# Hunger-Prevails/3D-Pose-Estimation-with-Previleged-Information

Measured on AMD Instinct MI355X. Metric: crops/sec (fwd+bwd) ResNet-50 pose head, 256x256 bs=64/GPU, higher is better.
Workload: dtype f32 (3xbf16 split, 6 products, f32 accumulate); 1 GPU; depthnet resnet50 pose head, 256x256 crops, batch 64/GPU, full step: fwd + soft-argmax + SmoothL1 + bwd + RCCL grad all-reduce + clip + Adam; global_batch=64, parallelism=dp1, dist_world_size=1, wgrad_stream_runs_beside_launch_stream=True

## Files before the change

### 3d-pose-estimation-with-previleged-information_amd/csrc/p3d_fx.hip

```cpp
#include <type_traits>
#include <mutex>
#include "p3d_common.h"
#include "p3d_fx.h"

namespace p3d {

using bf8 = __bf16 __attribute__((ext_vector_type(8)));
using f32x16 = float __attribute__((ext_vector_type(16)));
using f32x4 = float __attribute__((ext_vector_type(4)));
using f32x2 = float __attribute__((ext_vector_type(2)));
using u32x2 = unsigned __attribute__((ext_vector_type(2)));
using s4t = short __attribute__((ext_vector_type(4)));
using s8v = short __attribute__((ext_vector_type(8)));
using i32x4 = int __attribute__((ext_vector_type(4)));

constexpr int FX_BM = 128, FX_BN = 128, FX_BK = 16;
constexpr int FX_PIECE = 128 * FX_BK * 2;

using bf16x2 = __bf16 __attribute__((ext_vector_type(2)));
__device__ __forceinline__ unsigned fx_pack2(float a, float b) {
    const bf16x2 h = __builtin_convertvector(f32x2{a, b}, bf16x2);
    return __builtin_bit_cast(unsigned, h);
}
__device__ __forceinline__ void fx_split2(float x0, float x1, unsigned& hp, unsigned& mp, unsigned& lp) {
    hp = fx_pack2(x0, x1);
    const float r0 = x0 - __builtin_bit_cast(float, hp << 16), r1 = x1 - __builtin_bit_cast(float, hp & 0xFFFF0000u);
    mp = fx_pack2(r0, r1);
    const float s0 = r0 - __builtin_bit_cast(float, mp << 16), s1 = r1 - __builtin_bit_cast(float, mp & 0xFFFF0000u);
    lp = fx_pack2(s0, s1);
}
__device__ __forceinline__ void fx_split_store(unsigned char* base, const f32x4 v) {
    unsigned hp[2], mp[2], lp[2];
#pragma unroll
    for (int q = 0; q < 2; ++q) fx_split2(v[2 * q], v[2 * q + 1], hp[q], mp[q], lp[q]);
    *reinterpret_cast<u32x2*>(base) = u32x2{hp[0], hp[1]};
    *reinterpret_cast<u32x2*>(base + FX_PIECE) = u32x2{mp[0], mp[1]};
    *reinterpret_cast<u32x2*>(base + 2 * FX_PIECE) = u32x2{lp[0], lp[1]};
}

__device__ __forceinline__ int fx_tr_off(int row, int ch) { return 256 * row + 16 * (ch ^ (((row & 3) << 2) | ((row >> 2) & 3))); }
__device__ __forceinline__ int fx_rc_off(int row, int half) { return 32 * row + 16 * (half ^ ((row >> 3) & 1)); }

#define P3D_FX_PRODUCTS_AB(ACC, PIX, CH, NA, NB) P3D_FX_PRODUCTS_RANGE(ACC, PIX, CH, NA, NB, 0, 6)
#define P3D_FX_PRODUCTS_RANGE(ACC, PIX, CH, NA, NB, P0, P1)                                                            \
    _Pragma("unroll") for (int pa = P0; pa < P1; ++pa) {                                                               \
        constexpr int PP[6] = {2, 0, 1, 1, 0, 0}, PC[6] = {0, 2, 1, 0, 1, 0};                                           \
        _Pragma("unroll") for (int a = 0; a < NA; ++a) _Pragma("unroll") for (int b = 0; b < NB; ++b)                   \
            ACC[a][b] = __builtin_amdgcn_mfma_f32_32x32x16_bf16(PIX[PP[pa]][a], CH[PC[pa]][b], ACC[a][b], 0, 0, 0);    \
    }
__device__ __forceinline__ int fx_live_subtiles(int first, int limit) {
    const int n = (limit - first + 31) >> 5;
    return __builtin_amdgcn_readfirstlane(n < 0 ? 0 : (n > 2 ? 2 : n));
}

constexpr int FX_OOB = (int)0x80000000;
#if (defined(P3D_FX_ABL_NOLOAD) || defined(P3D_FX_ABL_NOREAD) || defined(P3D_FX_ABL_NOSTAGE) || defined(P3D_FX_ABL_NOBAR)) && !defined(P3D_TIMING_ONLY_BUILD)
#error "P3D_FX_ABL_* builds compute wrong results: define P3D_TIMING_ONLY_BUILD as well (tools/ablate.sh does) and never ship the library"
#endif
#ifdef P3D_FX_ABL_NOLOAD
#define FX_SO(x) 0
#else
#define FX_SO(x) (x)
#endif
#ifdef P3D_FX_ABL_NOREAD
#define FX_ABL_READ(kt) ((kt) == 0)
#else
#define FX_ABL_READ(kt) true
#endif
__device__ f32x4 fx_buffer_load_f32x4(i32x4 rsrc, int voffset, int soffset, int aux) __asm("llvm.amdgcn.raw.buffer.load.v4f32");
__device__ i32x4 fx_buffer_load_i32x4(i32x4 rsrc, int voffset, int soffset, int aux) __asm("llvm.amdgcn.raw.buffer.load.v4i32");
__device__ float fx_buffer_load_f32(i32x4 rsrc, int voffset, int soffset, int aux) __asm("llvm.amdgcn.raw.buffer.load.f32");
__device__ __forceinline__ i32x4 fx_rsrc(const void* base, size_t bytes) {
    const unsigned n = bytes < (size_t)0x80000000u ? (unsigned)bytes : 0x80000000u;
    const uint64_t a = reinterpret_cast<uint64_t>(base);
    i32x4 r;
    r[0] = (int)(unsigned)a; r[1] = (int)((a >> 32) & 0xffff); r[2] = (int)n; r[3] = 0x00020000;
    return r;
}
__device__ __forceinline__ bf8 fx_tr_read(const unsigned char* base, const int (&off)[2]) {
    s8v v;
#pragma unroll
    for (int half = 0; half < 2; ++half) {
        const s4t r4 = __builtin_amdgcn_ds_read_tr16_b64_v4i16((__attribute__((address_space(3))) s4t*)(base + off[half]));
#pragma unroll
        for (int e = 0; e < 4; ++e) v[4 * half + e] = r4[e];
    }
    return __builtin_bit_cast(bf8, v);
}
__device__ __forceinline__ void fx_tr_frag_off(int lane, int cb, int (&off)[2]) {
    const int g = lane >> 4, idx = lane & 15, q = idx >> 2, pq = idx & 3;
#pragma unroll
    for (int half = 0; half < 2; ++half) {
        const int row = 8 * (g >> 1) + 4 * half + q;
        off[half] = fx_tr_off(row, ((cb + 16 * (g & 1)) >> 3) + (pq >> 1)) + 8 * (pq & 1);
    }
}

__device__ __forceinline__ FxConvParams fx_class_params(const FxConvParams& in) {
    FxConvParams p = in;
    if (in.ncls > 0) {
        const FxConvClass& c = in.cls[blockIdx.z];
        p.nR = c.nR; p.nS = c.nS; p.ntap = c.ntap; p.r0 = c.r0; p.rstep = c.rstep; p.s0 = c.s0; p.sstep = c.sstep;
        p.hoff = c.hoff; p.hstep = c.hstep; p.woff = c.woff; p.wstep = c.wstep; p.oy0 = c.oy0; p.ox0 = c.ox0;
    }
    return p;
}

template <int AMODE, int PRO, int EPIX, bool TAPI = false>
__global__ __launch_bounds__(256, 3) void fx_conv_kernel(const FxConvParams p_in) {
    static_assert(!TAPI || AMODE == 1, "the tap-inner K order is an image-fed instance");
    constexpr int EPI = EPIX == 5 ? 1 : EPIX == 6 ? 2 : EPIX == 7 || EPIX == 8 ? 0 : EPIX;
    constexpr bool EM = EPIX == 4 || (EPIX >= 5 && EPIX <= 7);
    const FxConvParams p = fx_class_params(p_in);
    static_assert(AMODE == 0 || PRO == 0, "the partial-convolution factor is applied by the in-kernel split");
    __shared__ __attribute__((aligned(16))) unsigned char lds[2 * 6 * FX_PIECE];
    constexpr int BUFB = 6 * FX_PIECE, CH0 = 3 * FX_PIECE;
    float (*const red)[2][128] = reinterpret_cast<float (*)[2][128]>(lds + 40960);
    const int t = threadIdx.x, lane = t & 63, wave = __builtin_amdgcn_readfirstlane(t >> 6), wm = wave >> 1, wn = wave & 1;
    int bid;
    {
        const int nwg = gridDim.x, q = nwg >> 3, r = nwg & 7, xcd = blockIdx.x & 7, idx = blockIdx.x >> 3;
        bid = (xcd < r ? xcd * (q + 1) : r * (q + 1) + (xcd - r) * q) + idx;
    }
    const int tiles_n_all = gridDim.x / p.tiles_m;
    const int tile_m = p.order ? bid / tiles_n_all : bid % p.tiles_m, tile_n = p.order ? bid % tiles_n_all : bid / p.tiles_m;
    const int m0 = tile_m * FX_BM, n0 = tile_n * FX_BN;
    const int OHW = p.OH * p.OW;
    const int HWi = p.Hi * p.Wi;
    const int nfirst = n0 / OHW;
    const int csteps = p.Cred / FX_BK;
    int nk = p.ntap * csteps, kt0 = 0;
    if (p.kchunk > 0) {
        kt0 = blockIdx.y * p.kchunk;
        nk = min(nk - kt0, p.kchunk);
    }
    int f_tap = kt0 / csteps, f_k = (kt0 - f_tap * csteps) * FX_BK;
    if constexpr (TAPI) { f_k = (kt0 / p.ntap) * FX_BK; f_tap = kt0 - (kt0 / p.ntap) * p.ntap; }

    const i32x4 rW = fx_rsrc(p.Wimg, (size_t)p.R * p.S * p.tiles_m * csteps * (3 * FX_PIECE));
    int w_voff[3];
#pragma unroll
    for (int j = 0; j < 3; ++j) w_voff[j] = 16 * (t + 256 * j);

    const int trow = t >> 5, tp4 = t & 31;
    const int pp = t >> 1, ph = (t & 1) ^ ((t >> 4) & 1);
    const int col = n0 + (AMODE == 0 ? 4 * tp4 : pp);
    const bool col_ok = col < p.NP;
    int hbase = 0, wbase = 0, img_off = 0, mimg_off = 0;
    {
        const int cc = col_ok ? col : 0;
        const int pn = cc / OHW;
        const int rem = cc - pn * OHW, oh = rem / p.OW, ow = rem - oh * p.OW;
        hbase = oh * p.hmul + p.hoff;
        wbase = ow * p.wmul + p.woff;
// ... 569 lines not shown
                    for (int e = 0; e < 4; ++e) dst[e * p.oxs] = p.accumulate ? dst[e * p.oxs] + v[e] : v[e];
                }
            }
            if constexpr (EPI == 1) {
                if (!split) {
#pragma unroll
                    for (int e = 0; e < 4; ++e) { ssum[b] += v[e]; ssq[b] = fmaf(v[e], v[e], ssq[b]); }
                }
            }
            if constexpr (EPI == 2) {
                if (!split) {
                    const f32x4 c2 = *reinterpret_cast<const f32x4*>(p.ep_c + ((size_t)n * p.M + m) * OHW + rem);
#pragma unroll
                    for (int e = 0; e < 4; ++e) {
                        const float gg = fmaf(c2[e], esc[b], esh[b]) > 0.f ? v[e] : 0.f;
                        ssum[b] += gg; ssq[b] = fmaf(gg, c2[e] - emean[b], ssq[b]);
                    }
                }
            }
        }
    }
    if (dense) {
        constexpr int EROW = 512 + 16;
        constexpr int ROUNDS = (GB + 1) / 2;
        const bool accum = !split && p.accumulate;
#pragma unroll
        for (int r = 0; r < ROUNDS; ++r) {
            if (r > 0) __syncthreads();
#pragma unroll
            for (int b2 = 0; b2 < 2; ++b2) {
                const int b = 2 * r + b2;
                if (b < GB) {
#pragma unroll
                    for (int a = 0; a < GA; ++a)
                        *reinterpret_cast<f32x4*>(lds + (wm * 32 + b2 * 16 + lc) * EROW + (wn * 64 + a * 16 + 4 * lq) * 4) = acc[a][b < GB ? b : 0];
                }
            }
            __syncthreads();
#pragma unroll
            for (int i = 0; i < 8; ++i) {
                const int id = t + 256 * i, row = id >> 5, q = id & 31;
                const int within = r * 32 + (row & 31);
                const int m = m0 + (row >> 5) * WCH + within;
                const int c4 = n0 + 4 * q;
                if (within >= WCH || m >= p.M || c4 >= p.NP) continue;
                const int n = c4 / OHW, rem = c4 - n * OHW;
                f32x4 v = *reinterpret_cast<const f32x4*>(lds + row * EROW + q * 16);
                const size_t at = ((size_t)n * p.M + m) * OHW + rem;
                f32x4* dst = reinterpret_cast<f32x4*>(yout + at);
                if (accum) {
                    f32x4 o4;
                    if (p.acc_src) {
                        o4 = *reinterpret_cast<const f32x4*>(p.acc_src + at);
                        if (p.acc_mask) {
                            const unsigned mk = p.acc_mask[at >> 2];
#pragma unroll
                            for (int e = 0; e < 4; ++e) o4[e] = (mk >> e) & 1u ? o4[e] : 0.f;
                        }
                    } else o4 = *dst;
                    v[0] += o4[0]; v[1] += o4[1]; v[2] += o4[2]; v[3] += o4[3];
                }
                if constexpr (EPI == 8) {
                    if (p.ep_res) { const f32x4 r4 = *reinterpret_cast<const f32x4*>(p.ep_res + at); v[0] += r4[0]; v[1] += r4[1]; v[2] += r4[2]; v[3] += r4[3]; }
                    if (p.ep_relu) { v[0] = fmaxf(v[0], 0.f); v[1] = fmaxf(v[1], 0.f); v[2] = fmaxf(v[2], 0.f); v[3] = fmaxf(v[3], 0.f); }
                }
                *dst = v;
            }
        }
    }
    if constexpr (EPI == 1 || EPI == 2) {
        if (!split) {
#pragma unroll
            for (int b = 0; b < GB; ++b) {
                ssum[b] += __shfl_xor(ssum[b], 16, 64); ssq[b] += __shfl_xor(ssq[b], 16, 64);
                ssum[b] += __shfl_xor(ssum[b], 32, 64); ssq[b] += __shfl_xor(ssq[b], 32, 64);
                if (lq == 0) { red[wn][0][wm * WCH + b * 16 + lc] = ssum[b]; red[wn][1][wm * WCH + b * 16 + lc] = ssq[b]; }
            }
            __syncthreads();
            if (t < BM && m0 + t < p.M) {
                float* dst = p.partial + ((size_t)tile_n * p.M + m0 + t) * 2;
                dst[0] = red[0][0][t] + red[1][0][t];
                dst[1] = red[0][1][t] + red[1][1][t];
            }
        }
    }
}

template <int EPI>
__global__ __launch_bounds__(256) void fx_reduce_kernel(const float* __restrict__ slabs, float* __restrict__ y, const float* __restrict__ bias, int nsplit,
                                                        size_t slab_stride, int N, int M, int OHW, int accumulate, const float* __restrict__ ep_c,
                                                        const float* __restrict__ ep_tab, float* __restrict__ partial, const float* __restrict__ emask,
                                                        const float* __restrict__ res, int relu) {
    const int m = blockIdx.x, grp = blockIdx.y, ngrp = gridDim.y;
    const float bb = bias ? bias[m] : 0.f;
    float esc = 0.f, esh = 0.f, emean = 0.f;
    if constexpr (EPI == 2) { esc = ep_tab[8 * m]; esh = ep_tab[8 * m + 1]; emean = ep_tab[8 * m + 2]; }
    float s1 = 0.f, s2 = 0.f;
    const int q4 = OHW >> 2;
    for (int n = grp; n < N; n += ngrp) {
        const size_t base = ((size_t)n * M + m) * OHW;
        for (int i = threadIdx.x; i < q4; i += 256) {
            f32x4 v = *reinterpret_cast<const f32x4*>(slabs + base + 4 * i);
            for (int z = 1; z < nsplit; ++z) {
                const f32x4 u = *reinterpret_cast<const f32x4*>(slabs + (size_t)z * slab_stride + base + 4 * i);
                v[0] += u[0]; v[1] += u[1]; v[2] += u[2]; v[3] += u[3];
            }
            v[0] += bb; v[1] += bb; v[2] += bb; v[3] += bb;
            if (emask) {
                const f32x4 em = *reinterpret_cast<const f32x4*>(emask + (size_t)n * OHW + 4 * i);
                v[0] *= em[0]; v[1] *= em[1]; v[2] *= em[2]; v[3] *= em[3];
            }
            f32x4* dst = reinterpret_cast<f32x4*>(y + base + 4 * i);
            if (accumulate) { const f32x4 o = *dst; v[0] += o[0]; v[1] += o[1]; v[2] += o[2]; v[3] += o[3]; }
            if (res) { const f32x4 r4 = *reinterpret_cast<const f32x4*>(res + base + 4 * i); v[0] += r4[0]; v[1] += r4[1]; v[2] += r4[2]; v[3] += r4[3]; }
            if (relu) { v[0] = fmaxf(v[0], 0.f); v[1] = fmaxf(v[1], 0.f); v[2] = fmaxf(v[2], 0.f); v[3] = fmaxf(v[3], 0.f); }
            *dst = v;
            if constexpr (EPI == 1) {
#pragma unroll
                for (int e = 0; e < 4; ++e) { s1 += v[e]; s2 = fmaf(v[e], v[e], s2); }
            }
            if constexpr (EPI == 2) {
                const f32x4 c2 = *reinterpret_cast<const f32x4*>(ep_c + base + 4 * i);
#pragma unroll
                for (int e = 0; e < 4; ++e) { const float gg = fmaf(c2[e], esc, esh) > 0.f ? v[e] : 0.f; s1 += gg; s2 = fmaf(gg, c2[e] - emean, s2); }
            }
        }
    }
    if constexpr (EPI != 0) {
        __shared__ float r1[4], r2[4];
        s1 = wave_sum(s1); s2 = wave_sum(s2);
        if ((threadIdx.x & 63) == 0) { r1[threadIdx.x >> 6] = s1; r2[threadIdx.x >> 6] = s2; }
        __syncthreads();
        if (threadIdx.x == 0) {
            float* dst = partial + ((size_t)grp * M + m) * 2;
            dst[0] = r1[0] + r1[1] + r1[2] + r1[3];
            dst[1] = r2[0] + r2[1] + r2[2] + r2[3];
        }
    }
}

template <bool AIMG, bool BIMG, bool MASKED, int TAPS = 0>
__global__ __launch_bounds__(256, 3) void fx_wgrad_kernel(const FxWgradParams p) {
    static_assert(TAPS < 2 || (AIMG && BIMG && !MASKED), "the multi-tap column tiles are image-fed instances");
    static_assert(!MASKED || !AIMG || !BIMG, "the partial-convolution factors are applied by the in-kernel split of an fp32 operand (an image carries its factor already)");
    static_assert(!TAPS || BIMG, "tap-major columns come from an image operand");
    __shared__ __attribute__((aligned(16))) unsigned char As[2 * 3 * FX_PIECE];
    __shared__ __attribute__((aligned(16))) unsigned char Bs[2 * 3 * FX_PIECE];
    const int t = threadIdx.x, lane = t & 63, wave = t >> 6, wm = wave >> 1, wn = wave & 1;
    int bx, by, bz;
    {
        const int gx = gridDim.x, gy = gridDim.y, nwg = gx * gy * gridDim.z;
        const int lin = blockIdx.x + gx * (blockIdx.y + gy * blockIdx.z);
        const int q = nwg >> 3, r = nwg & 7, xcd = lin & 7, idx = lin >> 3;
        const int bid = (xcd < r ? xcd * (q + 1) : r * (q + 1) + (xcd - r) * q) + idx;
        if (p.order == 0 || TAPS) {
            bx = bid % gx;
            const int rest = bid / gx;
            by = rest % gy;
            bz = rest / gy;
        } else {
            const int nt = p.R * p.S;
            const int tp = bid % nt;
            int rest = bid / nt;
            by = rest % gy; rest /= gy;
            bx = rest % gx;
            bz = (rest / gx) * nt + tp;
// ... 499 lines not shown
    FxFinalize f{};
    if (fin) {
        f = *fin;
        if (!((f.kind == 1 && mode == 1 && f.beta) || ((f.kind == 2 || f.kind == 3) && mode == 2 && f.dgamma && f.dbeta)) || !f.partial || f.rows <= 0 || !f.gamma || !f.table) {
            set_error("fx_act_image: inconsistent fused-finalize request (kind %d, mode %d)", f.kind, mode); return P3D_EINVAL;
        }
    }
    const size_t plane = (size_t)N * C * HW * 2;
    const dim3 grid((unsigned)ceil_div((int64_t)N * (HW >> 2) * 2, 256), (unsigned)(C >> 4));
    if (mode == 0) hipLaunchKernelGGL(fx_act_image_kernel<0>, grid, dim3(256), 0, st, x, x2, table, (unsigned char*)img, plane, N, C, HW, masked, f, pixmul);
    else if (mode == 1) hipLaunchKernelGGL(fx_act_image_kernel<1>, grid, dim3(256), 0, st, x, x2, table, (unsigned char*)img, plane, N, C, HW, masked, f, pixmul);
    else hipLaunchKernelGGL(fx_act_image_kernel<2>, grid, dim3(256), 0, st, x, x2, table, (unsigned char*)img, plane, N, C, HW, masked, f, pixmul);
    return check_launch("fx_act_image");
}

static int g_fx = -1;
bool fx_enabled() {
    if (g_fx < 0) { const char* e = getenv("P3D_X3"); g_fx = (e && atoi(e) == 0) ? 0 : 1; }
    return g_fx == 1;
}
int fx_set_enabled(int on) { const int before = fx_enabled() ? 1 : 0; g_fx = on ? 1 : 0; return before; }

static std::mutex g_fx_count_mu;
static unsigned long long g_fx_count[6];
static double g_fx_flops[6];
void fx_count(int kind, const p3d_conv_desc* d) {
    std::lock_guard<std::mutex> lock(g_fx_count_mu);
    g_fx_count[kind] += 1;
    g_fx_flops[kind] += 2.0 * d->N * d->K * d->Ho * d->Wo * (double)d->C * d->R * d->S;
}
void fx_stats(unsigned long long* counts, double* flops, int reset) {
    std::lock_guard<std::mutex> lock(g_fx_count_mu);
    for (int i = 0; i < 6; ++i) { if (counts) counts[i] = g_fx_count[i]; if (flops) flops[i] = g_fx_flops[i]; }
    if (reset) for (int i = 0; i < 6; ++i) { g_fx_count[i] = 0; g_fx_flops[i] = 0.0; }
}

static bool fx_common(const p3d_conv_desc* d) {
    return fx_enabled() && d->c_offset >= 0 && d->c_offset + d->C <= d->c_total && d->R == d->S && (d->R & 1) && d->stride <= 2 &&
           (int64_t)d->N * d->C * d->H * d->W < (1ll << 31) && (int64_t)d->N * d->K * d->Ho * d->Wo < (1ll << 31) &&
           (int64_t)(d->K + 127) * (d->C + 127) * d->R * d->S * 6 < (1ll << 31);
}
bool fx_fwd_applies(const p3d_conv_desc* d, int min_m) {
    return fx_common(d) && d->C % FX_BK == 0 && d->C >= 32 && d->Wo % 4 == 0 && d->W % 4 == 0 && d->K >= min_m;
}
bool fx_dgrad_applies(const p3d_conv_desc* d, int min_m) {
    if (!(fx_common(d) && d->K % FX_BK == 0 && d->K >= 32 && d->C % 4 == 0 && d->C >= min_m && d->Wo % 4 == 0)) return false;
    if (d->stride == 1) return d->W % 4 == 0;
    return d->H % 2 == 0 && d->W % 8 == 0 && d->pad == d->dil * (d->R - 1) / 2 && (d->R == 1 || d->dil == 1);
}
bool fx_wgrad_applies(const p3d_conv_desc* d, int min_m) {
    if ((int64_t)d->N * d->C * d->H * d->W >= (1ll << 29) || (int64_t)d->N * d->K * d->Ho * d->Wo >= (1ll << 29)) return false;
    return fx_common(d) && d->K >= min_m && d->C >= min_m && (d->Ho * d->Wo) % FX_BK == 0 && d->Wo % 4 == 0 && d->W % 4 == 0 && (d->R == 1 || d->C % 64 == 0);
}

static int g_force_conv_splits = 0, g_force_wgrad_splits = 0, g_wgrad_target = 0;
static int g_tap_inner_min = [] { const char* e = getenv("P3D_TAP_INNER_MIN"); return e ? atoi(e) : 1024; }();
static int g_two_taps = 1;
static int g_conv_order = -1, g_wgrad_order = -1;
static int fx_conv_order(size_t wimg_bytes, int tiles_m, int tiles_n) {
    (void)wimg_bytes; (void)tiles_m; (void)tiles_n;
    return g_conv_order > 0 ? 1 : 0;
}
static int fx_wgrad_order(const p3d_conv_desc* d) {
    static const int env = [] { const char* e = getenv("P3D_WGRAD_ORDER"); return e ? atoi(e) : -1; }();
    const int forced = g_wgrad_order >= 0 ? g_wgrad_order : env;
    if (forced >= 0) return forced > 0 ? 1 : 0;
    return (d->R * d->S > 1 && d->C >= 512) ? 1 : 0;
}
static int g_class_launches = 0;
static int g_fx16 = -1;
static int fx16_mode() {
    if (g_fx16 < 0) { const char* e = getenv("P3D_FX16"); g_fx16 = e ? atoi(e) : 1; if (g_fx16 < 0 || g_fx16 > 2) g_fx16 = 1; }
    return g_fx16;
}
static int fx16_bm(int M, bool img, int pro, int epi) {
    const int mode = fx16_mode();
    if (epi == 5 || epi == 6 || epi == 7) epi = epi == 7 ? 0 : epi - 4;
    if (epi == 8) epi = 0;
    if (!img || pro != 0 || (epi != 0 && epi != 1 && epi != 2) || mode == 0) return 0;
    if (M <= 64) return 64;
    if (ceil_div(M, 96) * 96 < ceil_div(M, 128) * 128) return 96;
    return mode == 2 ? 128 : 0;
}
void fx_tune(int what, int value) {
    if (what == 3) { g_pair_map = value; return; }
    if (what == 5) { g_class_launches = value ? 1 : 0; return; }
    if (what == 9) { g_two_taps = value < 0 ? 1 : value; return; }
    if (what == 10) { g_tap_inner_min = value; return; }
    if (what == 7) { g_conv_order = value; return; }
    if (what == 8) { g_wgrad_order = value; return; }
    if (what == 4) { g_fx16 = value < 0 || value > 2 ? 1 : value; return; }
    (what == 0 ? g_force_wgrad_splits : what == 1 ? g_force_conv_splits : g_wgrad_target) = value;
}

struct FxSplit { int splits, kchunk; };
static FxSplit fx_plan_split(int64_t tiles, int nk) {
    FxSplit s{1, 0};
    int64_t want;
    if (g_force_conv_splits > 0) want = g_force_conv_splits < nk ? g_force_conv_splits : nk;
    else {
        static const int target = [] { const char* e = getenv("P3D_SPLITK_BLOCKS"); const int v = e ? atoi(e) : -1; return v >= 0 ? v : 768; }();
        if (tiles > 400 || nk < 64 || target == 0) return s;
        want = ceil_div(target, tiles);
        if (want > nk / 32) want = nk / 32;
        if (want > 8) want = 8;
    }
    if (want < 2) return s;
    s.kchunk = (int)ceil_div(nk, want);
    s.splits = (int)ceil_div(nk, s.kchunk);
    if (s.splits < 2) { s.splits = 1; s.kchunk = 0; }
    return s;
}

size_t fx_weight_image_bytes(int K, int C, int RS, bool bwd) {
    const int rows = bwd ? C : K, red = bwd ? K : C;
    return (size_t)RS * ((rows + 127) / 128) * (red / FX_BK) * (3 * FX_PIECE);
}
static size_t align256(size_t v) { return (v + 255) & ~(size_t)255; }

static FxSplit fx_fwd_split(const p3d_conv_desc* d) {
    return fx_plan_split(ceil_div(d->K, FX_BM) * ceil_div((int64_t)d->N * d->Ho * d->Wo, FX_BN), d->R * d->S * (d->C / FX_BK));
}
static FxSplit fx_dgrad_split(const p3d_conv_desc* d) {
    if (d->stride != 1) return FxSplit{1, 0};
    return fx_plan_split(ceil_div(d->C, FX_BM) * ceil_div((int64_t)d->N * d->H * d->W, FX_BN), d->R * d->S * (d->K / FX_BK));
}
static bool fx_masked_on() { static const bool on = [] { const char* e = getenv("P3D_FX_MASKED"); return !(e && atoi(e) == 0); }(); return on; }
bool fx_fwd_masked_applies(const p3d_conv_desc* d) { return fx_masked_on() && fx_fwd_applies(d, 64); }
bool fx_dgrad_masked_applies(const p3d_conv_desc* d) { return fx_masked_on() && fx_dgrad_applies(d, 64); }
bool fx_wgrad_masked_applies(const p3d_conv_desc* d) { return fx_masked_on() && fx_wgrad_applies(d, 96); }
size_t fx_fwd_workspace(const p3d_conv_desc* d) {
    const FxSplit s = fx_fwd_split(d);
    return align256(fx_weight_image_bytes(d->K, d->C, d->R * d->S, false)) + (s.splits > 1 ? (size_t)s.splits * d->N * d->K * d->Ho * d->Wo * sizeof(float) : 0);
}
size_t fx_dgrad_workspace(const p3d_conv_desc* d) {
    const FxSplit s = fx_dgrad_split(d);
    return align256(fx_weight_image_bytes(d->K, d->C, d->R * d->S, true)) + (s.splits > 1 ? (size_t)s.splits * d->N * d->C * d->H * d->W * sizeof(float) : 0);
}
int fx_partial_rows_fwd(const p3d_conv_desc* d) {
    const FxSplit s = fx_fwd_split(d);
    return s.splits > 1 ? (d->N < 16 ? d->N : 16) : (int)ceil_div((int64_t)d->N * d->Ho * d->Wo, FX_BN);
}
int fx_partial_rows_dgrad(const p3d_conv_desc* d) {
    const FxSplit s = fx_dgrad_split(d);
    return s.splits > 1 ? (d->N < 16 ? d->N : 16) : (int)ceil_div((int64_t)d->N * d->H * d->W, FX_BN);
}

__device__ __forceinline__ void fx_weight_image_chunks(const float* __restrict__ w, unsigned char* __restrict__ img, int K, int C, int RS, bool bwd, size_t first, size_t step,
                                                       int ctot, int coff, const float* __restrict__ scale = nullptr) {
    const int rows = bwd ? C : K, red = bwd ? K : C;
    const int tiles = (rows + 127) / 128, ksteps = red / FX_BK;
    const size_t total = (size_t)RS * tiles * ksteps * 256;
    for (size_t i = first; i < total; i += step) {
        const int half = (int)(i & 1), row = (int)((i >> 1) & 127);
        size_t j = i >> 8;
        const int ks = (int)(j % ksteps); j /= ksteps;
        const int tm = (int)(j % tiles);
        const int tap = (int)(j / tiles);
        const int m = tm * 128 + row, k0 = ks * FX_BK + half * 8;
        unsigned hi[8], mid[8], lo[8];
#pragma unroll
        for (int e = 0; e < 8; ++e) {
            float x = 0.f;
            if (m < rows) x = bwd ? w[((size_t)(k0 + e) * ctot + coff + m) * RS + tap] : w[((size_t)m * ctot + coff + k0 + e) * RS + tap];
            if (scale && m < rows) x = x * scale[m];
            const unsigned hb = __builtin_bit_cast(unsigned, x) & 0xFFFF0000u;
            const float r1 = x - __builtin_bit_cast(float, hb);
// ... 95 lines not shown
    const int am = img ? 1 : 0;
    FxConvParams p = p_in;
    if (p.tap_inner && !((bm == 0 && am == 1 && pro == 0 && epi >= 0 && epi <= 2) || (bm == 96 && epi >= 0 && epi <= 2))) p.tap_inner = 0;
    if (p.tap_inner) {
#define P3D_FX_TAPI(EPI) if (bm == 0 && epi == EPI) { hipLaunchKernelGGL((fx_conv_kernel<1, 0, EPI, true>), grid, dim3(256), 0, st, p); return; } \
                         if (bm == 96 && epi == EPI) { hipLaunchKernelGGL((fx16_conv_kernel<96, EPI, true>), grid, dim3(256), 0, st, p); return; }
        P3D_FX_TAPI(0) P3D_FX_TAPI(1) P3D_FX_TAPI(2)
#undef P3D_FX_TAPI
    }
#define P3D_FX16_CASE(BM, EPI) if (bm == BM && (epi == EPI || epi == (EPI == 0 ? 7 : EPI + 4))) { hipLaunchKernelGGL((fx16_conv_kernel<BM, EPI>), grid, dim3(256), 0, st, p); return; }
    P3D_FX16_CASE(128, 0) P3D_FX16_CASE(128, 1) P3D_FX16_CASE(128, 2)
    P3D_FX16_CASE(96, 0) P3D_FX16_CASE(96, 1) P3D_FX16_CASE(96, 2)
    P3D_FX16_CASE(64, 0) P3D_FX16_CASE(64, 1) P3D_FX16_CASE(64, 2)
    P3D_FX16_CASE(128, 8) P3D_FX16_CASE(96, 8) P3D_FX16_CASE(64, 8)
#undef P3D_FX16_CASE
#define P3D_FX_CASE(AM, PRO, EPI) if (am == AM && pro == PRO && epi == EPI) { hipLaunchKernelGGL((fx_conv_kernel<AM, PRO, EPI>), grid, dim3(256), 0, st, p); return; }
    P3D_FX_CASE(0, 0, 0) P3D_FX_CASE(0, 0, 1) P3D_FX_CASE(0, 0, 2) P3D_FX_CASE(0, 4, 0) P3D_FX_CASE(0, 4, 4) P3D_FX_CASE(0, 4, 5)
    P3D_FX_CASE(1, 0, 0) P3D_FX_CASE(1, 0, 1) P3D_FX_CASE(1, 0, 2) P3D_FX_CASE(1, 0, 3) P3D_FX_CASE(1, 0, 5) P3D_FX_CASE(1, 0, 6) P3D_FX_CASE(1, 0, 7)
    P3D_FX_CASE(0, 0, 8) P3D_FX_CASE(1, 0, 8)
#undef P3D_FX_CASE
    set_error("fx_launch_conv: no kernel instance for img=%d pro=%d epi=%d bm=%d", am, pro, epi, bm);
}

static void fx_launch_reduce(int epi, dim3 grid, hipStream_t st, const float* slabs, float* y, const float* bias, int nsplit, size_t slab_stride, int N, int M,
                             int OHW, int accumulate, const float* ep_c, const float* ep_tab, float* partial, const float* emask, const float* res = nullptr,
                             int relu = 0) {
    if (epi == 5 || epi == 6 || epi == 7 || epi == 4 || epi == 8) epi = epi == 5 ? 1 : epi == 6 ? 2 : 0;
    prof_kernel_done(st);
    if (epi == 1) hipLaunchKernelGGL(fx_reduce_kernel<1>, grid, dim3(256), 0, st, slabs, y, bias, nsplit, slab_stride, N, M, OHW, accumulate, ep_c, ep_tab, partial, emask, res, relu);
    else if (epi == 2) hipLaunchKernelGGL(fx_reduce_kernel<2>, grid, dim3(256), 0, st, slabs, y, bias, nsplit, slab_stride, N, M, OHW, accumulate, ep_c, ep_tab, partial, emask, res, relu);
    else hipLaunchKernelGGL(fx_reduce_kernel<0>, grid, dim3(256), 0, st, slabs, y, bias, nsplit, slab_stride, N, M, OHW, accumulate, ep_c, ep_tab, partial, emask, res, relu);
}

int32_t fx_conv_fwd(const p3d_conv_desc* d, const float* x, const float* w, const float* bias, float* y, void* workspace, size_t workspace_bytes,
                    const FxFuse* fuse, hipStream_t st) {
    const bool img = fuse && fuse->act_img;
    const bool masked = fuse && (fuse->pmask || fuse->emask);
    const bool infer = fuse && fuse->infer;
    const void* wimg = fuse ? fuse->wimg : nullptr;
    if (masked && (!fuse->emask || bias || (img ? fuse->pmask != nullptr : fuse->pmask == nullptr))) {
        set_error("fx_conv_fwd: the partial-convolution instances take the output factor, the input factor exactly for an fp32 operand, and no bias"); return P3D_EINVAL;
    }
    P3D_REQUIRE(!wimg || (d->c_offset == 0 && d->c_total == d->C), "fx_conv_fwd: a cached weight image with a channel window (c_offset %d, c_total %d, C %d)",
                d->c_offset, d->c_total, d->C);
    P3D_REQUIRE(!infer || (!masked && !fuse->partial && wimg), "fx_conv_fwd: the inference epilogue takes a cached folded weight image and no other fusion");
    P3D_REQUIRE(!(fuse && (fuse->res || fuse->relu)) || infer, "fx_conv_fwd: a residual / ReLU needs the inference epilogue");
    const size_t need = fx_fwd_workspace(d);
    if (need && (!workspace || workspace_bytes < need)) { set_error("fx_conv_fwd: workspace %zu B < required %zu B", workspace_bytes, need); return P3D_EWORKSPACE; }
    FxConvParams p{};
    p.X = x; p.Y = y; p.bias = bias;
    if (img) { p.Ximg = (const unsigned char*)fuse->act_img; p.plane_bytes = (size_t)d->N * d->C * d->H * d->W * 2; }
    p.N = d->N; p.Cred = d->C; p.Hi = d->H; p.Wi = d->W; p.M = d->K; p.OH = d->Ho; p.OW = d->Wo; p.NP = d->N * d->Ho * d->Wo;
    p.YH = d->Ho; p.YW = d->Wo; p.oy0 = 0; p.ox0 = 0; p.oys = 1; p.oxs = 1;
    p.R = d->R; p.S = d->S; p.nR = d->R; p.nS = d->S; p.ntap = d->R * d->S; p.r0 = 0; p.rstep = 1; p.s0 = 0; p.sstep = 1;
    p.hmul = d->stride; p.hoff = -d->pad; p.hstep = d->dil; p.wmul = d->stride; p.woff = -d->pad; p.wstep = d->dil;
    p.accumulate = d->accumulate;
    const int RS = d->R * d->S;
    char* ws = (char*)workspace;
    if (!wimg) {
        if (int32_t e = fx_build_weight_images(w, d->K, d->C, RS, ws, nullptr, st, d->c_total, d->c_offset)) return e;
        wimg = ws;
    }
    ws += align256(fx_weight_image_bytes(d->K, d->C, RS, false));
    p.Wimg = (const unsigned char*)wimg;
    int pro = 0, epi = 0;
    if (fuse) {
        if (fuse->partial) { epi = 1; p.partial = fuse->partial; }
        if (masked) { pro = img ? 0 : 4; epi = fuse->partial ? 5 : (img ? 7 : 4); p.pmask = fuse->pmask; p.emask = fuse->emask; }
        if (infer) { epi = 8; p.ep_res = fuse->res; p.ep_relu = fuse->relu; }
    }
    const int tiles_n = (int)ceil_div(p.NP, FX_BN);
    const FxSplit sp = fx_fwd_split(d);
    const int bm = fx16_bm(d->K, img, sp.splits > 1 ? 0 : pro, sp.splits > 1 ? 0 : epi);
    p.tiles_m = (int)ceil_div(d->K, bm ? bm : FX_BM);
    p.order = fx_conv_order(fx_weight_image_bytes(d->K, d->C, RS, false), p.tiles_m, tiles_n);
    p.tap_inner = img && RS > 1 && g_tap_inner_min > 0 && d->C >= g_tap_inner_min;
    if (sp.splits > 1) {
        p.kchunk = sp.kchunk; p.slab_stride = (size_t)d->N * d->K * d->Ho * d->Wo; p.Y = (float*)ws; p.bias = nullptr;
        const float* em = p.emask;
        p.emask = nullptr;
        fx_launch_conv(p, img, pro == 4 ? 4 : 0, 0, bm, dim3((unsigned)(p.tiles_m * tiles_n), (unsigned)sp.splits), st);
        fx_launch_reduce(epi, dim3((unsigned)d->K, (unsigned)(d->N < 16 ? d->N : 16)), st, (const float*)ws, y, bias, sp.splits, p.slab_stride, d->N, d->K,
                         d->Ho * d->Wo, d->accumulate, nullptr, nullptr, p.partial, em, p.ep_res, p.ep_relu);
    } else {
        fx_launch_conv(p, img, pro, epi, bm, dim3((unsigned)(p.tiles_m * tiles_n), 1), st);
    }
    return check_launch("fx_conv_fwd");
}

int32_t fx_conv_dgrad(const p3d_conv_desc* d, const float* dy, const float* w, float* dx, void* workspace, size_t workspace_bytes, const FxFuse* fuse,
                      hipStream_t st) {
    const bool img = fuse && fuse->act_img;
    const bool masked = fuse && (fuse->pmask || fuse->emask);
    const void* wimg = fuse ? fuse->wimg : nullptr;
    P3D_REQUIRE(!wimg || (d->c_offset == 0 && d->c_total == d->C), "fx_conv_dgrad: a cached weight image with a channel window (c_offset %d, c_total %d, C %d)",
                d->c_offset, d->c_total, d->C);
    if (masked && (!fuse->emask || (img ? fuse->pmask != nullptr : fuse->pmask == nullptr) || (!img && fuse->partial))) {
        set_error("fx_conv_dgrad: the partial-convolution instances take the result factor and the operand factor exactly for an fp32 operand"); return P3D_EINVAL;
    }
    const size_t need = fx_dgrad_workspace(d);
    if (need && (!workspace || workspace_bytes < need)) { set_error("fx_conv_dgrad: workspace %zu B < required %zu B", workspace_bytes, need); return P3D_EWORKSPACE; }
    if (fuse && fuse->acc_src && !(d->accumulate && fx_dgrad_accumulates_from_source(d))) {
        set_error("fx_conv_dgrad: an accumulation source needs accumulate = 1, stride 1 and an unsplit launch"); return P3D_EINVAL;
    }
    FxConvParams p{};
    p.X = dy; p.Y = dx;
    if (img) { p.Ximg = (const unsigned char*)fuse->act_img; p.plane_bytes = (size_t)d->N * d->K * d->Ho * d->Wo * 2; }
    p.N = d->N; p.Cred = d->K; p.Hi = d->Ho; p.Wi = d->Wo; p.M = d->C;
    p.YH = d->H; p.YW = d->W;
    p.R = d->R; p.S = d->S;
    p.accumulate = d->accumulate;
    const int RS = d->R * d->S;
    char* ws = (char*)workspace;
    if (!wimg) {
        if (int32_t e = fx_build_weight_images(w, d->K, d->C, RS, nullptr, ws, st, d->c_total, d->c_offset)) return e;
        wimg = ws;
    }
    ws += align256(fx_weight_image_bytes(d->K, d->C, RS, true));
    p.Wimg = (const unsigned char*)wimg;
    int pro = 0, epi = 0;
    if (fuse) {
        if (fuse->partial) { epi = 2; p.partial = fuse->partial; p.ep_c = fuse->ep_c; p.ep_tab = fuse->ep_tab; }
        if (masked) { pro = img ? 0 : 4; epi = fuse->partial ? 6 : (img ? 7 : 4); p.pmask = fuse->pmask; p.emask = fuse->emask; }
    }
    const bool dsplit = d->stride == 1 && fx_dgrad_split(d).splits > 1;
    static const int tap_inner_bwd = [] { const char* e = getenv("P3D_TAP_INNER_MIN_BWD"); return e ? atoi(e) : -1; }();
    const int ti_min = tap_inner_bwd >= 0 ? tap_inner_bwd : g_tap_inner_min;
    p.tap_inner = img && RS > 1 && ti_min > 0 && d->K >= ti_min;
    if (fuse && fuse->tail_c) {
        if (!(img && epi == 0 && pro == 0 && fx_dgrad_tail_applies(d) && fuse->tail_tab && fuse->tail_partial && (!fuse->tail_rc || fuse->tail_rtab))) {
            set_error("fx_conv_dgrad: the tail sums need an image-fed, dense, unsplit stride-1 data gradient without a BatchNorm epilogue (fx_dgrad_tail_applies)"); return P3D_EINVAL;
        }
        epi = 3;
        p.tail_c = fuse->tail_c; p.tail_tab = fuse->tail_tab; p.tail_rc = fuse->tail_rc; p.tail_rtab = fuse->tail_rtab; p.tail_mask = fuse->tail_mask; p.tail_partial = fuse->tail_partial;
    }
    const int bm = fx16_bm(d->C, img, dsplit ? 0 : pro, dsplit ? 0 : epi);
    p.tiles_m = (int)ceil_div(d->C, bm ? bm : FX_BM);
    if (d->stride == 1) {
        p.OH = d->H; p.OW = d->W; p.NP = d->N * d->H * d->W; p.oy0 = 0; p.ox0 = 0; p.oys = 1; p.oxs = 1;
        p.nR = d->R; p.nS = d->S; p.ntap = RS; p.r0 = 0; p.rstep = 1; p.s0 = 0; p.sstep = 1;
        p.hmul = 1; p.hoff = d->pad; p.hstep = -d->dil; p.wmul = 1; p.woff = d->pad; p.wstep = -d->dil;
        const int tiles_n = (int)ceil_div(p.NP, FX_BN);
        const FxSplit sp = fx_dgrad_split(d);
        p.order = fx_conv_order(fx_weight_image_bytes(d->K, d->C, RS, true), p.tiles_m, tiles_n);
        if (sp.splits > 1) {
            p.kchunk = sp.kchunk; p.slab_stride = (size_t)d->N * d->C * d->H * d->W; p.Y = (float*)ws;
            const float* em = p.emask;
            p.emask = nullptr;
            fx_launch_conv(p, img, pro == 4 ? 4 : 0, 0, bm, dim3((unsigned)(p.tiles_m * tiles_n), (unsigned)sp.splits), st);
            fx_launch_reduce(epi, dim3((unsigned)d->C, (unsigned)(d->N < 16 ? d->N : 16)), st, (const float*)ws, dx, nullptr, sp.splits, p.slab_stride, d->N, d->C,
                             d->H * d->W, d->accumulate, p.ep_c, p.ep_tab, p.partial, em);
        } else {
            if (fuse && fuse->acc_src && d->accumulate) { p.acc_src = fuse->acc_src; p.acc_mask = fuse->acc_mask; }
            fx_launch_conv(p, img, pro, epi, bm, dim3((unsigned)(p.tiles_m * tiles_n), 1), st);
        }
        return check_launch("fx_conv_dgrad");
    }
    if (epi != 0 && epi != 4 && epi != 7) { set_error("fx_conv_dgrad: the BatchNorm-backward epilogue is not available for strided data gradients"); return P3D_EINVAL; }
    const int st2 = d->stride;
    p.OH = d->H / st2; p.OW = d->W / st2; p.NP = d->N * p.OH * p.OW; p.oys = st2; p.oxs = st2;
    p.hmul = 1; p.wmul = 1;
    const int tiles_n = (int)ceil_div(p.NP, FX_BN);
    FxConvClass cls[4];
    int ncls = 0;
    for (int ph = 0; ph < st2; ++ph)
        for (int pw = 0; pw < st2; ++pw) {
            int nr = 0, ns = 0, r0 = -1, r1 = -1, q0 = -1, q1 = -1;
            for (int r = 0; r < d->R; ++r) { const int tt = ph + d->pad - r * d->dil; if (((tt % st2) + st2) % st2 == 0) { if (r0 < 0) r0 = r; else if (r1 < 0) r1 = r; ++nr; } }
            for (int s = 0; s < d->S; ++s) { const int tt = pw + d->pad - s * d->dil; if (((tt % st2) + st2) % st2 == 0) { if (q0 < 0) q0 = s; else if (q1 < 0) q1 = s; ++ns; } }
            if (nr == 0 || ns == 0) continue;
            FxConvParams c = p;
            c.nR = nr; c.nS = ns; c.ntap = nr * ns; c.r0 = r0; c.rstep = r1 < 0 ? 1 : r1 - r0; c.s0 = q0; c.sstep = q1 < 0 ? 1 : q1 - q0;
            const int th = ph + d->pad - r0 * d->dil, tw = pw + d->pad - q0 * d->dil;
            c.hoff = th >= 0 ? th / st2 : -((-th) / st2); c.hstep = -(c.rstep * d->dil) / st2;
            c.woff = tw >= 0 ? tw / st2 : -((-tw) / st2); c.wstep = -(c.sstep * d->dil) / st2;
            c.oy0 = ph; c.ox0 = pw;
            if (g_class_launches) { fx_launch_conv(c, img, pro, epi, bm, dim3((unsigned)(c.tiles_m * tiles_n), 1), st); continue; }
            cls[ncls++] = FxConvClass{c.nR, c.nS, c.ntap, c.r0, c.rstep, c.s0, c.sstep, c.hoff, c.hstep, c.woff, c.wstep, c.oy0, c.ox0};
        }
    if (ncls > 0) {
        for (int i = 1; i < ncls; ++i)
            for (int j = i; j > 0 && cls[j].ntap > cls[j - 1].ntap; --j) { const FxConvClass t = cls[j]; cls[j] = cls[j - 1]; cls[j - 1] = t; }
        p.ncls = ncls;
        for (int i = 0; i < ncls; ++i) p.cls[i] = cls[i];
        fx_launch_conv(p, img, pro, epi, bm, dim3((unsigned)(p.tiles_m * tiles_n), 1, (unsigned)ncls), st);
    }
    return check_launch("fx_conv_dgrad");
}

bool fx_dgrad_tail_applies(const p3d_conv_desc* d) {
    return fx_dgrad_applies(d, 96) && d->stride == 1 && fx_dgrad_split(d).splits == 1 && (d->H * d->W) % 4 == 0 && fx16_bm(d->C, true, 0, 0) == 0;
}
int fx_dgrad_tail_rows(const p3d_conv_desc* d) { return (int)ceil_div((int64_t)d->N * d->H * d->W, FX_BN); }
__global__ __launch_bounds__(64) void fx_tail_fold_kernel(const float* __restrict__ partial, int rows, int C, double* __restrict__ sums, int out_rows) {
    const int c = blockIdx.x * 64 + threadIdx.x, r = blockIdx.y;
    if (c >= C) return;
    double s0 = 0.0, s1 = 0.0, s2 = 0.0;
    for (int i = r; i < rows; i += out_rows) {
        const f32x4 v = *reinterpret_cast<const f32x4*>(partial + ((size_t)i * C + c) * 4);
        s0 += v[0]; s1 += v[1]; s2 += v[2];
    }
    double* dst = sums + ((size_t)c * out_rows + r) * 3;
    dst[0] = s0; dst[1] = s1; dst[2] = s2;
}
int32_t fx_tail_fold(const float* partial, int rows, int C, double* sums, int out_rows, hipStream_t st) {
    hipLaunchKernelGGL(fx_tail_fold_kernel, dim3((unsigned)ceil_div(C, 64), (unsigned)out_rows), dim3(64), 0, st, partial, rows, C, sums, out_rows);
    return check_launch("fx_tail_fold");
}

bool fx_dgrad_has_dead_classes(const p3d_conv_desc* d) { return d->stride > 1 && d->R == 1; }
bool fx_dgrad_accumulates_from_source(const p3d_conv_desc* d) { return d->stride == 1 && fx_dgrad_split(d).splits == 1 && (d->H * d->W) % 4 == 0; }

int fx_wgrad_two_taps(const p3d_conv_desc* d, bool images) {
    static const int env = [] { const char* e = getenv("P3D_TWO_TAPS"); return e ? atoi(e) : 1; }();
    if (!g_two_taps || !env || !images || d->C != 64 || d->R * d->S <= 1 || (d->Wo & 15)) return 0;
    return (g_two_taps == 1 && env == 1 && d->K <= 64) ? 3 : 2;
}
int fx_wgrad_splits(const p3d_conv_desc* d, bool images) {
    const int tt = fx_wgrad_two_taps(d, images);
    const int64_t tiles = tt ? ceil_div(d->K, FX_BM) * ceil_div(d->R * d->S, tt) : ceil_div(d->K, FX_BM) * ceil_div(d->C, FX_BN) * d->R * d->S;
    const int64_t total = (int64_t)d->N * (d->Ho * d->Wo / FX_BK);
    int64_t target;
    if (g_wgrad_target > 0) target = g_wgrad_target;
    else if (tiles >= 256) target = 1536;
    else switch ((int)tiles) {
        case 2: target = 384; break;
        case 4: target = 640; break;
        case 5: target = 512; break;
        case 8: case 32: case 36: target = 512; break;
        case 16: target = 256; break;
        case 128: target = 1024; break;
        case 144: target = 720; break;
        default: target = 768;
    }
    static const int scale = [] { const char* e = getenv("P3D_WGRAD_SCALE"); const int v = e ? atoi(e) : 0; return v > 0 ? v : 100; }();
    target = target * scale / 100;
    int64_t splits = (2 * target + tiles) / (2 * tiles);
// ... 188 lines not shown
```

Baseline: 2191 crops/s.

## Add short-K 1x1 conv kernel keeping activation tile resident across all M tiles

Adds a specialised kernel for 1x1 stride-1 convolutions with 64 reduction channels (e.g. ResNet bottleneck expand convs and their data gradients). Each block loads its 128-column activation tile (3 bf16 split planes) into LDS once and loops over every output-channel tile, streaming weights from global memory with a 4-deep register prefetch. The epilogue goes through LDS so stores are coalesced, with an optional BN-statistics partial. This removes repeated activation reloads across M tiles, at the cost of fewer, longer-running blocks and serialized M tiles within each block.

Result: no change. 2194 crops/s (median of 6 runs) (+0.1%).

```diff
diff --git a/3d-pose-estimation-with-previleged-information_amd/csrc/p3d_fx.hip b/3d-pose-estimation-with-previleged-information_amd/csrc/p3d_fx.hip
--- a/3d-pose-estimation-with-previleged-information_amd/csrc/p3d_fx.hip
+++ b/3d-pose-estimation-with-previleged-information_amd/csrc/p3d_fx.hip
@@ -70,6 +70,8 @@
 __device__ f32x4 fx_buffer_load_f32x4(i32x4 rsrc, int voffset, int soffset, int aux) __asm("llvm.amdgcn.raw.buffer.load.v4f32");
 __device__ i32x4 fx_buffer_load_i32x4(i32x4 rsrc, int voffset, int soffset, int aux) __asm("llvm.amdgcn.raw.buffer.load.v4i32");
 __device__ float fx_buffer_load_f32(i32x4 rsrc, int voffset, int soffset, int aux) __asm("llvm.amdgcn.raw.buffer.load.f32");
+__device__ void fx_buffer_store_f32x4(f32x4 v, i32x4 rsrc, int voffset, int soffset, int aux) __asm("llvm.amdgcn.raw.buffer.store.v4f32");
+__device__ void fx_buffer_store_f32x2(f32x2 v, i32x4 rsrc, int voffset, int soffset, int aux) __asm("llvm.amdgcn.raw.buffer.store.v2f32");
 __device__ __forceinline__ i32x4 fx_rsrc(const void* base, size_t bytes) {
     const unsigned n = bytes < (size_t)0x80000000u ? (unsigned)bytes : 0x80000000u;
     const uint64_t a = reinterpret_cast<uint64_t>(base);
@@ -805,6 +807,176 @@
                 dst[0] = red[0][0][t] + red[1][0][t];
                 dst[1] = red[0][1][t] + red[1][1][t];
             }
+        }
+    }
+}
+
+template <int CS, int EPI>
+__global__ __launch_bounds__(256, CS == 4 ? 2 : 1) void fx_conv_shortk_kernel(const FxConvParams p) {
+    static_assert(CS == 4 || CS == 8, "64 or 128 reduction channels");
+    static_assert(EPI == 0 || EPI == 1, "EPI 2 / 3 (their extra operands) spill at these register counts: those launches stay on fx_conv_kernel");
+    constexpr int ABYTES = CS * 3 * FX_PIECE, EBYTES = 64 * 512;
+    __shared__ __attribute__((aligned(16))) unsigned char lds[ABYTES + EBYTES];
+    unsigned char* const elds = lds + ABYTES;
+    const int t = threadIdx.x, lane = t & 63, wave = __builtin_amdgcn_readfirstlane(t >> 6), wm = wave >> 1, wn = wave & 1;
+    const int fr = lane & 31, fh = lane >> 5;
+    const int tile_n = blockIdx.x, n0 = tile_n * FX_BN;
+    const int OHW = p.OH * p.OW, HWi = p.Hi * p.Wi;
+    const int nfirst = n0 / OHW;
+
+    {
+        const int pp = t >> 1, ph = (t & 1) ^ ((t >> 4) & 1);
+        const int col = n0 + pp;
+        int voff = FX_OOB;
+        if (col < p.NP) {
+            const int pn = col / OHW, rem = col - pn * OHW;
+            voff = ((pn - nfirst) * CS * HWi + rem) * 32 + 16 * ph;
+        }
+        const size_t left = (size_t)(p.N - nfirst) * p.Cred * HWi * 2;
+        i32x4 rXi[3];
+#pragma unroll
+        for (int pc = 0; pc < 3; ++pc) rXi[pc] = fx_rsrc(p.Ximg + pc * p.plane_bytes + (size_t)nfirst * p.Cred * HWi * 2, left);
+        const int st = fx_rc_off(pp, ph);
+#pragma unroll
+        for (int h = 0; h < CS; h += 4) {
+            i32x4 v[4][3];
+#pragma unroll
+            for (int k = 0; k < 4; ++k)
+#pragma unroll
+                for (int pc = 0; pc < 3; ++pc) v[k][pc] = fx_buffer_load_i32x4(rXi[pc], voff, (h + k) * HWi * 32, 0);
+#pragma unroll
+            for (int k = 0; k < 4; ++k)
+#pragma unroll
+                for (int pc = 0; pc < 3; ++pc) *reinterpret_cast<i32x4*>(lds + ((h + k) * 3 + pc) * FX_PIECE + st) = v[k][pc];
+        }
+    }
+
+    const int nsteps = p.tiles_m * CS;
+    const i32x4 rW = fx_rsrc(p.Wimg, (size_t)nsteps * (3 * FX_PIECE));
+    int w_voff[3][2];
+#pragma unroll
+    for (int pc = 0; pc < 3; ++pc)
+#pragma unroll
+        for (int b = 0; b < 2; ++b) w_voff[pc][b] = pc * FX_PIECE + fx_rc_off(wm * 64 + b * 32 + fr, fh);
+    bf8 wf[4][3][2];
+    auto wfetch = [&](int slot, int s) {
+        const int so = (s < nsteps ? s : nsteps - 1) * (3 * FX_PIECE);
+#pragma unroll
+        for (int pc = 0; pc < 3; ++pc)
+#pragma unroll
+            for (int b = 0; b < 2; ++b) wf[slot][pc][b] = __builtin_bit_cast(bf8, fx_buffer_load_i32x4(rW, w_voff[pc][b], so, 0));
+    };
+#pragma unroll
+    for (int s = 0; s < 4; ++s) wfetch(s, s);
+    int rd_p[2];
+#pragma unroll
+    for (int a = 0; a < 2; ++a) rd_p[a] = fx_rc_off(wn * 64 + a * 32 + fr, fh);
+    __syncthreads();
+
+    float* const yout = p.Y;
+    const bool accum = p.accumulate;
+    const i32x4 rY = fx_rsrc(p.Y, (size_t)p.NP * p.M * sizeof(float));
+    const i32x4 rPart = fx_rsrc(p.partial, EPI == 1 ? (size_t)gridDim.x * p.M * 8 : 0);
+    for (int tm = 0; tm < p.tiles_m; ++tm) {
+        const int m0 = tm * FX_BM;
+        f32x16 acc[2][2];
+#pragma unroll
+        for (int a = 0; a < 2; ++a)
+#pragma unroll
+            for (int b = 0; b < 2; ++b)
+#pragma unroll
+                for (int r = 0; r < 16; ++r) acc[a][b][r] = 0.f;
+#pragma unroll
+        for (int kt = 0; kt < CS; ++kt) {
+            bf8 pf[3][2];
+#pragma unroll
+            for (int pc = 0; pc < 3; ++pc)
+#pragma unroll
+                for (int a = 0; a < 2; ++a) pf[pc][a] = *reinterpret_cast<const bf8*>(lds + (kt * 3 + pc) * FX_PIECE + rd_p[a]);
+            bf8 (&cf)[3][2] = wf[kt & 3];
+            P3D_FX_PRODUCTS_AB(acc, pf, cf, 2, 2)
+            __builtin_amdgcn_sched_barrier(0);
+            wfetch(kt & 3, tm * CS + kt + 4);
+            __builtin_amdgcn_sched_barrier(0);
+        }
+
+        float ssum[2] = {0.f, 0.f}, ssq[2] = {0.f, 0.f};
+        {
+#pragma unroll
+            for (int a = 0; a < 2; ++a)
+#pragma unroll
+                for (int g = 0; g < 4; ++g) {
+                    const int c4 = n0 + wn * 64 + a * 32 + 8 * g + 4 * fh;
+                    if (c4 >= p.NP) continue;
+#pragma unroll
+                    for (int b = 0; b < 2; ++b) {
+                        const int m = m0 + wm * 64 + b * 32 + fr;
+                        f32x4 v = {acc[a][b][4 * g], acc[a][b][4 * g + 1], acc[a][b][4 * g + 2], acc[a][b][4 * g + 3]};
+                        if (p.bias) { const float bb = p.bias[m]; v[0] += bb; v[1] += bb; v[2] += bb; v[3] += bb; }
+#pragma unroll
+                        for (int e = 0; e < 4; ++e) acc[a][b][4 * g + e] = v[e];
+                        if constexpr (EPI == 1) {
+#pragma unroll
+                            for (int e = 0; e < 4; ++e) { ssum[b] += v[e]; ssq[b] = fmaf(v[e], v[e], ssq[b]); }
+                        }
+                    }
+                }
+        }
+#pragma unroll
+        for (int b = 0; b < 2; ++b) {
+            __syncthreads();
+#pragma unroll
+            for (int a = 0; a < 2; ++a)
+#pragma unroll
+                for (int g = 0; g < 4; ++g) {
+                    const int row = wm * 32 + fr, q = wn * 16 + a * 8 + 2 * g + fh;
+                    *reinterpret_cast<f32x4*>(elds + row * 512 + ((q ^ (row & 7)) << 4)) =
+                        f32x4{acc[a][b][4 * g], acc[a][b][4 * g + 1], acc[a][b][4 * g + 2], acc[a][b][4 * g + 3]};
+                }
+            __syncthreads();
+#pragma unroll
+            for (int i = 0; i < 8; ++i) {
+                const int id = t + 256 * i, row = id >> 5, q = id & 31;
+                const int m = m0 + (row >> 5) * 64 + b * 32 + (row & 31);
+                const int c4 = n0 + 4 * q;
+                const bool ok = c4 < p.NP;
+                const int n = (ok ? c4 : 0) / OHW, rem = (ok ? c4 : 0) - n * OHW;
+                f32x4 v = *reinterpret_cast<const f32x4*>(elds + row * 512 + ((q ^ (row & 7)) << 4));
+                const int at = (n * p.M + m) * OHW + rem;
+                const f32x4* dst = reinterpret_cast<const f32x4*>(yout + at);
+                if (accum) {
+                    f32x4 o4;
+                    if (p.acc_src) {
+                        o4 = *reinterpret_cast<const f32x4*>(p.acc_src + at);
+                        if (p.acc_mask) {
+                            const unsigned mk = p.acc_mask[at >> 2];
+#pragma unroll
+                            for (int e = 0; e < 4; ++e) o4[e] = (mk >> e) & 1u ? o4[e] : 0.f;
+                        }
+                    } else o4 = *dst;
+                    v[0] += o4[0]; v[1] += o4[1]; v[2] += o4[2]; v[3] += o4[3];
+                }
+                fx_buffer_store_f32x4(v, rY, ok ? at * 4 : FX_OOB, 0, 0);
+            }
+        }
+        if constexpr (EPI == 1) {
+            float (*const red)[2][128] = reinterpret_cast<float (*)[2][128]>(elds);
+#pragma unroll
+            for (int b = 0; b < 2; ++b) {
+                ssum[b] += __shfl_xor(ssum[b], 32, 64);
+                ssq[b] += __shfl_xor(ssq[b], 32, 64);
+            }
+            __syncthreads();
+            if (fh == 0) {
+#pragma unroll
+                for (int b = 0; b < 2; ++b) {
+                    const int ch = wm * 64 + b * 32 + fr;
+                    red[wn][0][ch] = ssum[b]; red[wn][1][ch] = ssq[b];
+                }
+            }
+            __syncthreads();
+            const int ch = t & 127, po = t < 128 ? (tile_n * p.M + m0 + ch) * 8 : FX_OOB;
+            fx_buffer_store_f32x2(f32x2{red[0][0][ch] + red[1][0][ch], red[0][1][ch] + red[1][1][ch]}, rPart, po, 0, 0);
         }
     }
 }
@@ -1470,7 +1642,24 @@
     if (ceil_div(M, 96) * 96 < ceil_div(M, 128) * 128) return 96;
     return mode == 2 ? 128 : 0;
 }
+static int g_shortk = -1;
+static int fx_shortk_steps(const FxConvParams& p, bool img, int pro, int epi, int bm, bool split) {
+    if (g_shortk < 0) { const char* e = getenv("P3D_FX_SHORTK"); g_shortk = (e && atoi(e) == 0) ? 0 : 1; }
+    if (!g_shortk || !img || pro != 0 || (epi != 0 && epi != 1) || bm != 0 || split) return 0;
+    if (p.R != 1 || p.S != 1 || p.hmul != 1 || p.wmul != 1 || p.hoff != 0 || p.woff != 0 || p.OH != p.Hi || p.OW != p.Wi || p.ncls > 0) return 0;
+    if (p.YH != p.OH || p.YW != p.OW || p.oys != 1 || p.oxs != 1 || (p.OH * p.OW) % 4 != 0 || p.M % FX_BM != 0 || p.M < 2 * FX_BM) return 0;
+    if ((int64_t)p.NP * p.M * sizeof(float) >= (1ll << 31)) return 0;
+    return p.Cred == 64 ? 4 : 0;
+}
+static void fx_launch_shortk(const FxConvParams& p, int cs, int epi, hipStream_t st) {
+    const dim3 grid((unsigned)ceil_div(p.NP, FX_BN));
+#define P3D_FX_SK(CS, EPI) if (cs == CS && epi == EPI) { hipLaunchKernelGGL((fx_conv_shortk_kernel<CS, EPI>), grid, dim3(256), 0, st, p); return; }
+    P3D_FX_SK(4, 0) P3D_FX_SK(4, 1)
+#undef P3D_FX_SK
+    set_error("fx_launch_shortk: no kernel instance for cs=%d epi=%d", cs, epi);
+}
 void fx_tune(int what, int value) {
+    if (what == 11) { g_shortk = value < 0 ? -1 : (value ? 1 : 0); return; }
     if (what == 3) { g_pair_map = value; return; }
     if (what == 5) { g_class_launches = value ? 1 : 0; return; }
     if (what == 9) { g_two_taps = value < 0 ? 1 : value; return; }
@@ -1732,6 +1921,8 @@
         fx_launch_conv(p, img, pro == 4 ? 4 : 0, 0, bm, dim3((unsigned)(p.tiles_m * tiles_n), (unsigned)sp.splits), st);
         fx_launch_reduce(epi, dim3((unsigned)d->K, (unsigned)(d->N < 16 ? d->N : 16)), st, (const float*)ws, y, bias, sp.splits, p.slab_stride, d->N, d->K,
                          d->Ho * d->Wo, d->accumulate, nullptr, nullptr, p.partial, em, p.ep_res, p.ep_relu);
+    } else if (const int cs = fx_shortk_steps(p, img, pro, epi, bm, false)) {
+        fx_launch_shortk(p, cs, epi, st);
     } else {
         fx_launch_conv(p, img, pro, epi, bm, dim3((unsigned)(p.tiles_m * tiles_n), 1), st);
     }
@@ -1802,7 +1993,8 @@
                              d->H * d->W, d->accumulate, p.ep_c, p.ep_tab, p.partial, em);
         } else {
             if (fuse && fuse->acc_src && d->accumulate) { p.acc_src = fuse->acc_src; p.acc_mask = fuse->acc_mask; }
-            fx_launch_conv(p, img, pro, epi, bm, dim3((unsigned)(p.tiles_m * tiles_n), 1), st);
+            if (const int cs = fx_shortk_steps(p, img, pro, epi, bm, false)) fx_launch_shortk(p, cs, epi, st);
+            else fx_launch_conv(p, img, pro, epi, bm, dim3((unsigned)(p.tiles_m * tiles_n), 1), st);
         }
         return check_launch("fx_conv_dgrad");
     }
```
